# nemo110110/modify-sift-gpu

Hardware: AMD Instinct MI355X
Metric: SIFT images/sec at 1080p (features/sec alongside), 1/2/4/8 MI355X (higher is better)
Workload: dtype f32

## Files before the change

### include/sgpu.h

```cpp
#ifndef SGPU_H
#define SGPU_H
#include <stddef.h>
#include <stdint.h>

#ifdef __cplusplus
extern "C" {
#endif

#define SGPU_OK 0
#define SGPU_EINVAL (-1)
#define SGPU_ENODEV (-2)
#define SGPU_ENOMEM (-3)
#define SGPU_ERANGE (-4)

typedef struct sgpu_options {
    float filter_width_factor;
    float descriptor_window_factor;
    float orientation_window_factor;
    float orientation_gaussian_factor;
    float dog_threshold;
    float edge_threshold;
    int subpixel;
    int max_orientation;
    int fixed_orientation;
// ... 146 lines not shown
#define SGPU_DEBUG_GAUSS_BLOCK 32
#define SGPU_DEBUG_BAND_SHIFT 20
#define SGPU_DEBUG_KEYED_MATCH 64
#define SGPU_DEBUG_FULL_COLUMNS 128
#define SGPU_DEBUG_DESC_DUAL 256
#define SGPU_DEBUG_ORIENT_WAVE 512
#define SGPU_DEBUG_GAUSS_TILE_ALWAYS 1024
#define SGPU_DEBUG_MATCH_REGSTAGE 2048
#define SGPU_DEBUG_PYR_SERIAL 4096
#define SGPU_DEBUG_GAUSS_LONG_BANDS 8192
#define SGPU_DEBUG_DUO_ALWAYS 16384
#define SGPU_DEBUG_DUO_OFF 32768
#define SGPU_DEBUG_GAUSS_TILE_OFF 65536
#define SGPU_DEBUG_DESC_WIDE_OFF 131072
#define SGPU_DEBUG_DESC_WIDE_ALWAYS 262144
#define SGPU_DEBUG_EXTREMA_TILE_OFF 524288

int sgpu_debug_set_flags(sgpu_ctx* ctx, int flags);
#define SGPU_FEATURES_QUEUE 0
#define SGPU_FEATURES_STATIC_ORIENTATION 1
#define SGPU_FEATURES_STATIC_DESCRIPTOR 2
#define SGPU_FEATURES_STATIC 3
int sgpu_debug_set_feature_queue(sgpu_ctx* ctx, int mode);
#define SGPU_TRIO_OFF 0
#define SGPU_TRIO_ON 1
#define SGPU_TRIO_ALWAYS 2
#define SGPU_PAIRS_FRONT 0
#define SGPU_PAIRS_END 1
int sgpu_debug_set_schedule(sgpu_ctx* ctx, int trio, int pairs);
#define SGPU_DUO_STRIPS_RULE 0
#define SGPU_DUO_STRIPS_WAVE 1
#define SGPU_DUO_STRIPS_COOP 2
int sgpu_debug_set_duo_strips(sgpu_ctx* ctx, int mode);
int sgpu_debug_set_match_prune(sgpu_ctx* ctx, int on);
int sgpu_debug_match_plan_stats(const sgpu_ctx* ctx, long long out[4]);
#define SGPU_PLAN_ENTRY_INTS 7
#define SGPU_PLAN_LEVEL 0
#define SGPU_PLAN_TILE 1
#define SGPU_PLAN_TWO 2
#define SGPU_PLAN_TILE_TWO 3
#define SGPU_PLAN_TILE_DUO 4
#define SGPU_PLAN_TILE_DUO_ONE 5
#define SGPU_PLAN_DUO 6
#define SGPU_PLAN_TRIO 7
#define SGPU_PLAN_KINDS 8
int sgpu_debug_pyramid_plan(const sgpu_ctx* ctx, int* out, int cap);
int sgpu_debug_geometry(const sgpu_ctx* ctx, int* n_octaves, int* dims , int max);
int sgpu_debug_gaussian(sgpu_ctx* ctx, int image, int octave, int level, float* out);
int sgpu_debug_candidates(sgpu_ctx* ctx, int* ints, float* floats, int cap, int* n);

#ifdef __cplusplus
}
#endif
#endif
```

### modify-sift-gpu_amd/csrc/sgpu_capi.cpp

```cpp
#include <dlfcn.h>
#include <hip/hip_runtime.h>
#include <rccl/rccl.h>

#include <algorithm>
#include <cmath>
#include <cstdio>
#include <cstdlib>
#include <atomic>
#include <cstring>
#include <string>
#include <vector>

#include "../../include/sgpu.h"
#include "sift_kernels.h"
#include "sift_geom.h"
#include "sift_match_plan.h"
#include "sift_params.h"
#include "sift_pyramid_plan.h"

namespace {

#ifndef SGK_WIDE_DESC_MAX
#define SGK_WIDE_DESC_MAX 8192
#endif
// ... 63 lines not shown
            if (e) (void)hipEventDestroy(e);
        if (stream) (void)hipStreamDestroy(stream);
        if (stream_lo) (void)hipStreamDestroy(stream_lo);
        if (ev_ds) (void)hipEventDestroy(ev_ds);
        if (ev_oct) (void)hipEventDestroy(ev_oct);
        ev_ds = ev_oct = nullptr;
        if (stream_oct) (void)hipStreamDestroy(stream_oct);
        stream = stream_lo = stream_oct = nullptr;
    }
};

constexpr int kMaxParts = 4;
#ifndef SGPU_WAVE_ORIENT_MAX
#define SGPU_WAVE_ORIENT_MAX 16384
#endif
constexpr size_t kWaveOrientationMax = SGPU_WAVE_ORIENT_MAX;

}

struct sgpu_ctx {
    int device = 0;
    hipStream_t stream = nullptr;
    sgpu_options opt{};
    sgp::Schedule sched{};
    sgp::InputPlan plan{};
    int debug_flags = 0;
    bool multi_stream = false;
    bool duo_on = false;
    bool duo_wide = false;
    bool duo_u8 = false;
    int trio_mode = SGPU_TRIO_OFF;
    int duo_plan = SGK_DUO_PLAN;
    int duo_strips = SGPU_DUO_STRIPS_RULE;
    size_t wide_desc_max = SGK_WIDE_DESC_MAX;
    size_t wave_orient_max = kWaveOrientationMax;
    bool unit_input = true;
    bool tile_duo = false;
    int tile_mb = SGK_TILE_MB;
    int env_flags = 0;
    sgk::FeatureQueue fq{};
    bool queue_ori = true, queue_desc = true;
    struct HostOut {
        float* keys = nullptr;
        float* desc = nullptr;
        int cap = 0;
        bool armed = false, active = false, done = false;
    } host_out;
    bool stage_timing = true;
    bool streaming = false;
    std::string err;
    int batch = 0, w = 0, h = 0, nparts = 0;
    std::vector<sgp::Octave> oct;
    size_t staged_bytes = 0;
    std::vector<int64_t> img_off;
    Part part[kMaxParts];
    DevBuf input, all_keys, all_desc, gray, pre;
    DevBuf input2;
    DevBuf duo_trash;
    hipStream_t h2d = nullptr, d2h = nullptr;
    hipEvent_t up_ev[2] = {}, down_ev[2] = {};
    bool gathered = false;
    hipEvent_t ev[T_N + 1] = {};
    float timing[T_N] = {};
    DevBuf m_d1, m_d2, m_s1, m_s2, m_part, m_terms, m_match, m_dist, m_mask, m_loc, m_colpart, m_cols;
    DevBuf m_prune, m_s1c;
    bool match_prune = true;
// ... 169 lines not shown
    if (!pt.ev_ds) {
        for (hipEvent_t& e : pt.ev)
            if (hipEventCreate(&e) != hipSuccess) return SGPU_ENODEV;
        if (hipEventCreateWithFlags(&pt.ev_ds, hipEventDisableTiming) != hipSuccess ||
            hipEventCreateWithFlags(&pt.ev_oct, hipEventDisableTiming) != hipSuccess)
            return SGPU_ENODEV;
    }
    return SGPU_OK;
}

int sgpu_ctx_create(int device, const sgpu_options* opt, sgpu_ctx** out) {
    if (!out) return SGPU_EINVAL;
    *out = nullptr;
    int n = 0;
    if (hipGetDeviceCount(&n) != hipSuccess || n <= 0) return SGPU_ENODEV;
    if (device < 0 || device >= n) return SGPU_EINVAL;
    sgpu_ctx* ctx = new sgpu_ctx();
    ctx->device = device;
    if (hipSetDevice(device) != hipSuccess ||
        hipStreamCreateWithFlags(&ctx->stream, hipStreamNonBlocking) != hipSuccess) {
        delete ctx;
        return SGPU_ENODEV;
    }
    for (int i = 0; i <= T_N; i++) (void)hipEventCreate(&ctx->ev[i]);
    {
        Part* p = ctx->part;
        bool ok = part_streams(p[0], PS_MAIN) == SGPU_OK && part_streams(p[0], PS_OCT) == SGPU_OK &&
                  hipStreamCreateWithFlags(&ctx->h2d, hipStreamNonBlocking) == hipSuccess &&
                  hipStreamCreateWithFlags(&ctx->d2h, hipStreamNonBlocking) == hipSuccess &&
                  part_streams(p[0], PS_LO) == SGPU_OK && part_streams(p[1], PS_OCT) == SGPU_OK &&
                  part_streams(p[2], PS_MAIN) == SGPU_OK && part_streams(p[2], PS_LO) == SGPU_OK &&
                  part_streams(p[1], PS_MAIN) == SGPU_OK && part_streams(p[1], PS_LO) == SGPU_OK;
        ok = ok && sgk::feature_queue_grids(&ctx->fq) == hipSuccess;
        for (int i = 0; ok && i < 2; i++)
            ok = hipEventCreateWithFlags(&ctx->up_ev[i], hipEventDisableTiming) == hipSuccess &&
                 hipEventCreateWithFlags(&ctx->down_ev[i], hipEventDisableTiming) == hipSuccess;
        if (!ok) {
            sgpu_ctx_destroy(ctx);
            return SGPU_ENODEV;
        }
    }
    if (const char* ev = getenv("SGPU_EXACT_DESCRIPTOR"))
        if (ev[0] == '1') ctx->debug_flags |= SGPU_DEBUG_EXACT_DESCRIPTOR;
    if (const char* ev = getenv("SGPU_GAUSS")) {
        if (!strcmp(ev, "block")) ctx->debug_flags |= SGPU_DEBUG_GAUSS_BLOCK;
    }
    if (const char* ev = getenv("SGPU_DUO")) {
        if (!strcmp(ev, "off")) ctx->debug_flags |= SGPU_DEBUG_DUO_OFF;
        if (!strcmp(ev, "always")) ctx->debug_flags |= SGPU_DEBUG_DUO_ALWAYS;
        if (!strcmp(ev, "on")) ctx->duo_on = true;
    }
    if (const char* ev = getenv("SGPU_DUO_WIDE")) {
        if (ev[0] == '1') ctx->duo_wide = true;
    }
    if (const char* ev = getenv("SGPU_DUO_U8")) {
        if (ev[0] == '1') ctx->duo_u8 = true;
    }
    if (const char* ev = getenv("SGPU_DUO_PLAN")) {
        if (!strcmp(ev, "end")) ctx->duo_plan = SGPU_PAIRS_END;
        if (!strcmp(ev, "front")) ctx->duo_plan = SGPU_PAIRS_FRONT;
    }
    if (const char* ev = getenv("SGPU_TRIO")) {
        if (!strcmp(ev, "off")) ctx->trio_mode = SGPU_TRIO_OFF;
        if (!strcmp(ev, "always")) ctx->trio_mode = SGPU_TRIO_ALWAYS;
        if (!strcmp(ev, "on")) ctx->trio_mode = SGPU_TRIO_ON;
    }
    if (const char* ev = getenv("SGPU_GAUSS_BANDS"))
        if (!strcmp(ev, "long")) ctx->debug_flags |= SGPU_DEBUG_GAUSS_LONG_BANDS;
    if (const char* ev = getenv("SGPU_PYR")) {
        if (!strcmp(ev, "serial")) ctx->debug_flags |= SGPU_DEBUG_PYR_SERIAL;
    }
    if (const char* ev = getenv("SGPU_STREAMS")) ctx->multi_stream = !strcmp(ev, "multi");
    if (const char* ev = getenv("SGPU_MATCH"))
        if (!strcmp(ev, "reg")) ctx->debug_flags |= SGPU_DEBUG_MATCH_REGSTAGE;
    if (const char* ev = getenv("SGPU_DESC")) {
        if (!strcmp(ev, "dual")) ctx->debug_flags |= SGPU_DEBUG_DESC_DUAL;
        if (!strcmp(ev, "narrow")) ctx->debug_flags |= SGPU_DEBUG_DESC_WIDE_OFF;
        if (!strcmp(ev, "wide")) ctx->debug_flags |= SGPU_DEBUG_DESC_WIDE_ALWAYS;
    }
    if (const char* ev = getenv("SGPU_GAUSS_TILE")) {
        if (!strcmp(ev, "off")) ctx->debug_flags |= SGPU_DEBUG_GAUSS_TILE_OFF;
        if (!strcmp(ev, "always")) ctx->debug_flags |= SGPU_DEBUG_GAUSS_TILE_ALWAYS;
    }
    if (const char* ev = getenv("SGPU_WIDE_DESC_MAX"))
        if (atoll(ev) >= 0) ctx->wide_desc_max = (size_t)atoll(ev);
    if (const char* ev = getenv("SGPU_WAVE_ORIENT_MAX"))
        if (atoll(ev) >= 0) ctx->wave_orient_max = (size_t)atoll(ev);
    if (const char* ev = getenv("SGPU_EXTREMA")) {
        if (!strcmp(ev, "wave")) ctx->debug_flags |= SGPU_DEBUG_EXTREMA_TILE_OFF;
// ... 278 lines not shown
    auto rec = [&](int i, hipStream_t s_) -> hipError_t {
        return pt.events ? hipEventRecord(pt.ev[i], s_) : hipSuccess;
    };
    HIPCHK(ctx, rec(0, st));
    const size_t img_elems = (size_t)stride * h;
    const uint8_t* src8 = is_f32 ? nullptr : (const uint8_t*)src_in + (size_t)pt.img0 * img_elems;
    const float* srcf = is_f32 ? (const float*)src_in + (size_t)pt.img0 * img_elems : nullptr;

    float* pyr = pt.pyr.as<float>();
    const int rc_ops = build_level_ops(ctx, pt, src8, srcf, stride, st);
    if (rc_ops != SGPU_OK) return rc_ops;
    const sgpyr::Rules R = pyramid_rules(ctx, pt);
    sgpyr::plan_pyramid(pt.levels.data(), (int)pt.levels.size(), R, OpSupport{pt.ops.data()}, pt.plan);
    const int rc_trash = pt.plan.trash ? ensure_gauss_trash(ctx) : SGPU_OK;
    if (rc_trash != SGPU_OK) return rc_trash;
    const bool side = pt.plan.side;
    float* const trash = ctx->duo_trash.as<float>();
    pt.gauss_launches = 0;
    for (const sgpyr::Launch& l : pt.plan.launches) {
        const hipStream_t s_ = l.side ? pt.stream_oct : st;
        const sgk::LevelOp& a = pt.ops[l.op[0]];
        const sgk::LevelOp& b = pt.ops[std::max(l.op[1], 0)];
        const sgk::LevelOp& c = pt.ops[std::max(l.op[2], 0)];
        int nl = 1;
        if (l.wait_ds) HIPCHK(ctx, hipStreamWaitEvent(s_, pt.ev_ds, 0));
        switch (l.kind) {
            case sgpyr::kLevel: HIPCHK(ctx, sgk::launch_gauss_op(a, s_, R.wave_rows, R.long_bands)); break;
            case sgpyr::kTile: HIPCHK(ctx, sgk::launch_gauss_tile(a, s_)); break;
            case sgpyr::kTwo: HIPCHK(ctx, sgk::launch_gauss_two(a, b, s_, R.wave_rows, R.long_bands, &nl)); break;
            case sgpyr::kTileTwo: HIPCHK(ctx, sgk::launch_gauss_tile_two(a, b, s_, &nl)); break;
            case sgpyr::kTileDuo: HIPCHK(ctx, sgk::launch_gauss_tile_duo(a, b, s_)); break;
            case sgpyr::kTileDuoOne: HIPCHK(ctx, sgk::launch_gauss_tile_duo_one(a, b, c, s_, &nl)); break;
            case sgpyr::kDuo:
                HIPCHK(ctx, sgk::launch_gauss_duo(a, b, s_, R.wave_rows, trash, ctx->duo_strips));
                break;
            case sgpyr::kTrio: HIPCHK(ctx, sgk::launch_gauss_trio(a, b, c, s_, R.wave_rows, trash)); break;
            default: return ctx->fail(SGPU_EINVAL, "unknown pyramid launch kind");
        }
        pt.gauss_launches += nl;
        if (l.rec_ds) HIPCHK(ctx, hipEventRecord(pt.ev_ds, st));
    }
    if (side) {
        HIPCHK(ctx, hipEventRecord(pt.ev_oct, pt.stream_oct));
        HIPCHK(ctx, hipStreamWaitEvent(st, pt.ev_oct, 0));
    }
    HIPCHK(ctx, rec(1, st));

    if (!pt.one_stream)
        HIPCHK(ctx, sgk::launch_zero(pt.row_count.as<uint32_t>(), (size_t)pt.total_rows,
                                     pt.mask.as<uint32_t>(), (size_t)moff, nullptr, 0, st));
    const bool ext_tiles = !(ctx->debug_flags & SGPU_DEBUG_EXTREMA_TILE_OFF) &&
                           ((ctx->debug_flags & SGPU_DEBUG_GAUSS_TILE_ALWAYS) ||
                            4ll * fp.oct[0].wa * fp.oct[0].h * n <= ((long long)ctx->tile_mb << 20));
    HIPCHK(ctx, sgk::launch_extrema(pyr, pt.mask.as<uint32_t>(), pt.row_count.as<uint32_t>(),
                                    fp, st, ext_tiles));
    if (O.feature_count_threshold > 0)
        HIPCHK(ctx, sgk::launch_limit_rows(pt.row_count.as<uint32_t>(), fp,
                                           O.feature_count_threshold, O.truncate_method, st));
    HIPCHK(ctx, rec(7, st));
    HIPCHK(ctx, sgk::launch_scan(pt.row_count.as<uint32_t>(), pt.row_base.as<uint32_t>(),
                                 pt.total_rows, pt.scan_tmp.as<uint32_t>(), st));
    HIPCHK(ctx, rec(2, st));

    if (!pt.one_stream) {
        st = pt.stream_lo;
        HIPCHK(ctx, hipStreamWaitEvent(st, pt.ev[2], 0));
    }
// ... 1493 lines not shown
    out[0] = (long long)plan.items.size();
    out[1] = (long long)plan.sides.size();
    out[2] = tiles;
    out[3] = chunks;
    return SGPU_OK;
}

static_assert(SGPU_PLAN_KINDS == sgpyr::kKinds && SGPU_PLAN_TRIO == sgpyr::kTrio &&
              SGPU_PLAN_TILE_DUO_ONE == sgpyr::kTileDuoOne, "sgpu.h and sift_pyramid_plan.h agree");
int sgpu_debug_pyramid_plan(const sgpu_ctx* ctx, int* out, int cap) {
    if (!ctx || ctx->batch <= 0 || cap < 0 || (cap > 0 && !out)) return SGPU_EINVAL;
    const Part& pt = ctx->part[0];
    const int n = (int)pt.plan.launches.size();
    for (int e = 0; e < n && (e + 1) * SGPU_PLAN_ENTRY_INTS <= cap; e++) {
        const sgpyr::Launch& l = pt.plan.launches[e];
        int* p = out + e * SGPU_PLAN_ENTRY_INTS;
        p[0] = l.kind;
        for (int j = 0; j < 3; j++) {
            p[1 + 2 * j] = l.op[j] < 0 ? -1 : pt.levels[l.op[j]].o;
            p[2 + 2 * j] = l.op[j] < 0 ? -1 : pt.levels[l.op[j]].k;
        }
    }
    return n;
}

static_assert(SGPU_DUO_STRIPS_RULE == sgk::kDuoStripsRule && SGPU_DUO_STRIPS_WAVE == sgk::kDuoStripsWave &&
              SGPU_DUO_STRIPS_COOP == sgk::kDuoStripsCoop, "sgpu.h and sift_kernels.h agree");
int sgpu_debug_set_duo_strips(sgpu_ctx* ctx, int mode) {
    if (!ctx || mode < SGPU_DUO_STRIPS_RULE || mode > SGPU_DUO_STRIPS_COOP) return SGPU_EINVAL;
    ctx->duo_strips = mode;
    return SGPU_OK;
}

int sgpu_debug_set_feature_queue(sgpu_ctx* ctx, int mode) {
    if (!ctx || mode < SGPU_FEATURES_QUEUE || mode > SGPU_FEATURES_STATIC) return SGPU_EINVAL;
    ctx->queue_ori = !(mode & SGPU_FEATURES_STATIC_ORIENTATION);
    ctx->queue_desc = !(mode & SGPU_FEATURES_STATIC_DESCRIPTOR);
    return SGPU_OK;
}

int sgpu_debug_set_schedule(sgpu_ctx* ctx, int trio, int pairs) {
    if (!ctx || trio < SGPU_TRIO_OFF || trio > SGPU_TRIO_ALWAYS || pairs < SGPU_PAIRS_FRONT ||
        pairs > SGPU_PAIRS_END)
        return SGPU_EINVAL;
    ctx->trio_mode = trio;
    ctx->duo_plan = pairs;
    return SGPU_OK;
}

int sgpu_debug_geometry(const sgpu_ctx* ctx, int* n_octaves, int* dims, int max) {
    if (!ctx || !n_octaves) return SGPU_EINVAL;
    *n_octaves = (int)ctx->oct.size();
    for (int o = 0; o < (int)ctx->oct.size() && o < max; o++) {
        dims[3 * o] = ctx->oct[o].w;
        dims[3 * o + 1] = ctx->oct[o].h;
        dims[3 * o + 2] = ctx->oct[o].wa;
    }
    return SGPU_OK;
}

int sgpu_debug_gaussian(sgpu_ctx* ctx, int image, int octave, int level, float* out) {
    if (!ctx || image < 0 || image >= ctx->batch || octave < 0 ||
        octave >= (int)ctx->oct.size() || level < 0 || level >= ctx->sched.level_num)
        return SGPU_EINVAL;
    HIPCHK(ctx, hipSetDevice(ctx->device));
    const Part& pt = ctx->part[ctx->part_of(image)];
// ... 63 lines not shown
```

### modify-sift-gpu_amd/csrc/sift_gauss_duo.hip

```cpp
#include <cstdint>
#include <cstdlib>
#include <cstring>
#include <utility>

#include "sift_gauss_coop_plan.h"
#include "sift_gauss_ring.h"
#include "sift_kernels.h"
#include "sift_pyramid_plan.h"

#pragma clang diagnostic ignored "-Winline-asm"

namespace sgk {
namespace {

using namespace gring;

#ifndef SGK_DUO_INTERLEAVE
#define SGK_DUO_INTERLEAVE 1
#endif
constexpr bool kDuoInterleave = SGK_DUO_INTERLEAVE != 0;
#ifndef SGK_DUO_EXP
#define SGK_DUO_EXP 0
#endif
#ifndef SGK_DUO_X4
#define SGK_DUO_X4 1
#endif
constexpr int kDuoWaves = 4;
constexpr int kMidSlot = 256;
static_assert(kDuoWaves == coop::kWaves && 2 * coop::kWaveCols == kMidSlot, "cooperative geometry");

__device__ __forceinline__ void coop_barrier() {
    asm volatile("" ::: "memory");
    wait_lgkm0();
    __builtin_amdgcn_s_barrier();
    asm volatile("" ::: "memory");
}

// ... 490 lines not shown
        return e ? atoi(e) : SGK_DUO_NIN;
    }();
    return v == 5 ? 5 : v == 4 ? 4 : 7;
}
static int duo_bands_env() {
    static const int v = [] {
        const char* e = getenv("SGPU_DUO_BANDS");
        return e ? atoi(e) : 0;
    }();
    return v;
}
#ifndef SGK_DUO_WAVES
#define SGK_DUO_WAVES 4096
#endif
static long long duo_waves_target() {
    static const long long v = [] {
        const char* e = getenv("SGPU_DUO_WAVES");
        return e && atoll(e) > 0 ? atoll(e) : (long long)SGK_DUO_WAVES;
    }();
    return v;
}

template <int FWA, int FWB>
constexpr bool kDuoCoopCompiled = !(FWA == 17 && FWB == 21);
#ifndef SGK_DUO_COOP_RULE
#define SGK_DUO_COOP_RULE 1
#endif
#ifndef SGK_DUO_COOP_MAXW
#define SGK_DUO_COOP_MAXW 1920
#endif
template <int FWA, int FWB>
constexpr bool kDuoCoopRule = SGK_DUO_COOP_RULE != 0 && SGK_DUO_EXP == 0 && kDuoCoopCompiled<FWA, FWB>;

template <int FWA, int FWB, bool U8, int DS, bool COOP>
hipError_t duo_launch_form(const LevelOp& a, const LevelOp& b, hipStream_t stream, int rows_hint,
                           float* trash) {
    using G = DuoGeom<FWA, FWB>;
    DuoJob J{};
    J.src = a.src;
    J.src8 = a.src_u8;
    J.zero = a.zero;
    J.src_stride = a.src_stride;
    J.src_img = a.src_img_stride;
    J.dst1 = a.dst;
    J.dst2 = b.dst;
    J.dst_img = a.dst_img_stride;
    J.W = a.w;
    J.H = a.h;
    J.ta = a.taps;
    J.tb = b.taps;
    const LevelOp& dl = DS == 2 ? b : a;
    J.ds = dl.ds_dst;
    J.dsw = dl.ds_w;
    J.dsh = dl.ds_h;
    J.ds_img = dl.ds_img_stride;
    J.strips = COOP ? coop::strips(a.w, FWB) : (a.w + G::SW - 1) / G::SW;
    const long long per_band = (long long)J.strips * a.batch * (COOP ? kDuoWaves : 1);
    int nsy = 1;
    const long long want = duo_waves_target();
    if (rows_hint > 0) {
        nsy = (a.h + rows_hint - 1) / rows_hint;
    } else if (duo_bands_env() > 0) {
        nsy = std::min(duo_bands_env(), std::max(1, a.h / 64));
    } else if (per_band < want) {
        nsy = (int)std::min<long long>((want + per_band - 1) / per_band, std::max(1, a.h / 64));
    }
    int rows = (a.h + nsy - 1) / nsy;
    rows = (rows + 7) / 8 * 8;
    J.nsy = (a.h + rows - 1) / rows;
    J.rows_per_band = rows;
    J.total_waves = (int)(per_band * J.nsy);
    J.trash = trash;
    const unsigned nb = (unsigned)((J.total_waves + kDuoWaves - 1) / kDuoWaves);
    if constexpr (U8)
        hipLaunchKernelGGL((k_gauss_duo<FWA, FWB, 2, true, DS, COOP>), dim3(nb), dim3(64 * kDuoWaves), 0, stream, J);
    else if constexpr (COOP)
        hipLaunchKernelGGL((k_gauss_duo<FWA, FWB, 7, false, DS, true>), dim3(nb), dim3(64 * kDuoWaves), 0, stream, J);
    else if (duo_nin() == 5)
        hipLaunchKernelGGL((k_gauss_duo<FWA, FWB, 5, false, DS, false>), dim3(nb), dim3(64 * kDuoWaves), 0, stream, J);
    else if (duo_nin() == 4)
        hipLaunchKernelGGL((k_gauss_duo<FWA, FWB, 4, false, DS, false>), dim3(nb), dim3(64 * kDuoWaves), 0, stream, J);
    else
        hipLaunchKernelGGL((k_gauss_duo<FWA, FWB, 7, false, DS, false>), dim3(nb), dim3(64 * kDuoWaves), 0, stream, J);
    return hipGetLastError();
}

template <int FWA, int FWB, bool U8, int DS>
hipError_t duo_launch(const LevelOp& a, const LevelOp& b, hipStream_t stream, int rows_hint,
                      float* trash, int strips) {
    if constexpr (kDuoCoopCompiled<FWA, FWB>) {
        const bool rule = kDuoCoopRule<FWA, FWB> && a.w <= SGK_DUO_COOP_MAXW &&
                          coop::fewer_lane_columns(a.w, FWB);
        if (strips == kDuoStripsCoop || (strips == kDuoStripsRule && rule))
            return duo_launch_form<FWA, FWB, U8, DS, true>(a, b, stream, rows_hint, trash);
    }
    return duo_launch_form<FWA, FWB, U8, DS, false>(a, b, stream, rows_hint, trash);
}

}

bool gauss_duo_supported(const LevelOp& a, const LevelOp& b) {
    const bool u8 = a.src_u8 != nullptr;
    const bool ds = a.ds_dst != nullptr, dsb = b.ds_dst != nullptr;
    const bool widths = sgpyr::duo_widths(a.fw, b.fw, u8, ds, dsb);
    const bool dsb_ok = dsb && widths && (b.w % 2) == 0 && b.ds_w * 2 == b.w &&
                        (b.ds_h == (b.h + 1) / 2 || b.ds_h == b.h / 2) &&
                        b.ds_img_stride >= (long long)b.ds_w * b.ds_h;
    const bool dsa_ok = (a.w % 2) == 0 && a.ds_w * 2 == a.w && a.ds_h == (a.h + 1) / 2 &&
                        a.ds_img_stride >= (long long)a.ds_w * a.ds_h;
    const bool pair = widths && (!dsb || dsb_ok) && (u8 || dsb || !ds || dsa_ok);
    const bool src_ok = u8 ? (!a.src && (a.src_stride % 4) == 0 && (a.src_img_stride % 4) == 0 &&
                              ((uintptr_t)a.src_u8 % 4) == 0)
                           : (a.src && a.src_stride >= a.w);
    const bool b_zeroes = (b.zero.n[0] | b.zero.n[1] | b.zero.n[2]) != 0;
    const bool a_zeroes = (a.zero.n[0] | a.zero.n[1] | a.zero.n[2]) != 0;
    return pair && src_ok && !b_zeroes && (u8 || !a_zeroes) && (!b.ds_dst || dsb_ok) &&
           b.src == a.dst && !b.src_u8 && a.w == b.w && a.h == b.h && a.batch == b.batch &&
           a.w >= 8 && a.h >= 8 && (a.w % 4) == 0 && b.src_stride == a.w &&
           a.dst_img_stride == b.dst_img_stride && b.src_img_stride == a.dst_img_stride &&
           a.dst_img_stride >= (long long)a.w * a.h;
}

hipError_t launch_gauss_duo(const LevelOp& a, const LevelOp& b, hipStream_t stream, int rows_hint,
                            float* trash, int strips) {
    if (!trash || !gauss_duo_supported(a, b)) return hipErrorInvalidValue;
    if (a.src_u8) return duo_launch<13, 11, true, 0>(a, b, stream, rows_hint, trash, strips);
    if (a.ds_dst) return duo_launch<17, 21, false, 1>(a, b, stream, rows_hint, trash, strips);
    if (b.ds_dst) return duo_launch<13, 17, false, 2>(a, b, stream, rows_hint, trash, strips);
#define SGK_DUO(A, B) \
    if (a.fw == A && b.fw == B) return duo_launch<A, B, false, 0>(a, b, stream, rows_hint, trash, strips);
    SGK_DUO(11, 13) SGK_DUO(21, 25)
#undef SGK_DUO
    return hipErrorInvalidValue;
}

}
```

### modify-sift-gpu_amd/csrc/sift_kernels.h

```cpp
#pragma once
#include <hip/hip_runtime.h>
#include <stdint.h>

namespace sgk {

constexpr int kMaxLevels = 16;
constexpr int kMaxOctaves = 16;

struct Taps { float k[33]; };

struct OctaveDesc {
    int w, h, wa;
    int nwords;
    long long gauss_off;
    long long level_stride;
    long long mask_off;
    long long mask_level_stride;
};

struct FeatureParams {
    int batch, n_octaves, d;
    int rows_per_image;
    int row_off[kMaxOctaves];
    float level_sigma[kMaxLevels];
// ... 12 lines not shown
    uint32_t* p[3] = {nullptr, nullptr, nullptr};
    size_t n[3] = {0, 0, 0};
};

hipError_t launch_gauss(const float* src, const uint8_t* src_u8, int src_stride,
                        long long src_img_stride, float* dst, long long dst_img_stride,
                        int w, int h, int fw, const Taps& taps, int batch,
                        float* ds_dst, int ds_w, int ds_h, long long ds_img_stride,
                        hipStream_t stream, int wave_rows = -1, bool long_bands = false,
                        const ZeroJob& zero = ZeroJob{});

struct LevelOp {
    const float* src;
    const uint8_t* src_u8;
    int src_stride;
    long long src_img_stride;
    float* dst;
    long long dst_img_stride;
    int w, h, fw;
    Taps taps;
    int batch;
    float* ds_dst;
    int ds_w, ds_h;
    long long ds_img_stride;
    ZeroJob zero;
};
hipError_t launch_gauss_op(const LevelOp& op, hipStream_t stream, int wave_rows,
                           bool long_bands = false);
hipError_t launch_gauss_two(const LevelOp& a, const LevelOp& b, hipStream_t stream, int wave_rows,
                            bool long_bands = false, int* launches = nullptr);

constexpr size_t kGaussDuoTrashBytes = 1024 * 3072;
constexpr int kDuoStripsRule = 0, kDuoStripsWave = 1, kDuoStripsCoop = 2;
bool gauss_duo_supported(const LevelOp& a, const LevelOp& b);
hipError_t launch_gauss_duo(const LevelOp& a, const LevelOp& b, hipStream_t stream, int rows_hint,
                            float* trash, int strips = kDuoStripsRule);

constexpr size_t kGaussTrioTrashBytes = 1024 * 4096;
bool gauss_trio_supported(const LevelOp& a, const LevelOp& b, const LevelOp& c);
hipError_t launch_gauss_trio(const LevelOp& a, const LevelOp& b, const LevelOp& c,
                             hipStream_t stream, int rows_hint, float* trash);

bool gauss_tile_supported(const LevelOp& op);
hipError_t launch_gauss_tile(const LevelOp& op, hipStream_t stream);
hipError_t launch_gauss_tile_two(const LevelOp& a, const LevelOp& b, hipStream_t stream,
                                 int* launches = nullptr);
bool gauss_tile_duo_supported(const LevelOp& a, const LevelOp& b);
hipError_t launch_gauss_tile_duo(const LevelOp& a, const LevelOp& b, hipStream_t stream);
hipError_t launch_gauss_tile_duo_one(const LevelOp& a, const LevelOp& b, const LevelOp& c,
                                     hipStream_t stream, int* launches = nullptr);

hipError_t launch_first_octave_input(const float* src, const uint8_t* src_u8, int stride,
                                     long long src_img_stride, int tw, int h, int fo, float* dst,
                                     int dw, int dh, long long dst_img_stride, int batch,
                                     hipStream_t stream);

hipError_t launch_color_to_gray(const uint8_t* src, int n, int w, int h, int stride,
                                int channels, bool bgr, float* dst, hipStream_t stream);

hipError_t launch_extrema(const float* pyr, uint32_t* mask, uint32_t* row_count,
                          const FeatureParams& fp, hipStream_t stream, bool tiles = false);

size_t scan_tmp_words(size_t n);
hipError_t launch_zero(uint32_t* a, size_t na, uint32_t* b, size_t nb, uint32_t* c, size_t nc,
                       hipStream_t stream);
hipError_t launch_scan(const uint32_t* in, uint32_t* out, size_t n, uint32_t* tmp,
                       hipStream_t stream);

constexpr int kQueueCounters = 8;
// ... 154 lines not shown
```

### modify-sift-gpu_amd/python/sgpu.py

```python
from __future__ import annotations

import contextlib
import ctypes
import os
import subprocess

import numpy as np

from sgpu_types import SgpuOptions, default_options

PKG = os.path.dirname(os.path.dirname(os.path.abspath(__file__)))
LIB_PATH = os.environ.get("SGPU_LIB_PATH") or os.path.join(PKG, "lib", "libsiftgpu.so")

SGPU_OK, SGPU_EINVAL, SGPU_ENODEV, SGPU_ENOMEM, SGPU_ERANGE = 0, -1, -2, -3, -4
SGPU_INPUT_HOST, SGPU_INPUT_DEVICE, SGPU_INPUT_STAGED = 0, 1, 2

C_API = [
    "sgpu_default_options", "sgpu_parse_args", "sgpu_ctx_create", "sgpu_ctx_destroy",
    "sgpu_ctx_set_options", "sgpu_last_error", "sgpu_device_count", "sgpu_extract",
    "sgpu_extract_f32", "sgpu_stage_input", "sgpu_feature_count", "sgpu_feature_total", "sgpu_copy_features",
    "sgpu_device_features", "sgpu_match", "sgpu_quantize_descriptors", "sgpu_last_timing",
    "sgpu_debug_geometry", "sgpu_debug_gaussian", "sgpu_debug_candidates",
    "sgpu_debug_set_flags", "sgpu_comm_unique_id", "sgpu_comm_init", "sgpu_comm_allgather_i32",
    "sgpu_comm_allreduce_f64", "sgpu_extract_keypoints", "sgpu_match_guided", "sgpu_extract_color",
    "sgpu_match_shard_begin", "sgpu_match_shard_end", "sgpu_match_sharded",
    "sgpu_extract_stream", "sgpu_host_alloc", "sgpu_host_free", "sgpu_reserve",
    "sgpu_debug_alloc_count", "sgpu_last_pyramid_launches", "sgpu_set_stage_timing",
    "sgpu_set_host_output", "sgpu_debug_set_schedule", "sgpu_debug_set_match_prune",
    "sgpu_quantize_descriptors_gpu", "sgpu_feature_descriptors_u8", "sgpu_copy_features_u8",
    "sgpu_match_batch", "sgpu_match_images", "sgpu_debug_match_plan_stats",
    "sgpu_debug_set_duo_strips", "sgpu_debug_pyramid_plan", "sgpu_debug_set_feature_queue",
    "sgpu_match_batch_guided", "sgpu_match_images_guided",
    "sgpu_estimate_batch", "sgpu_estimate_images",
]

PLAN_KINDS = ("level", "tile", "two", "tile_two", "tile_duo", "tile_duo_one", "duo", "trio")

_LIB = None


def build():
    subprocess.check_call(["make", "-C", PKG, "-j8"])


def lib():
    global _LIB
    if _LIB is None:
        if not os.path.exists(LIB_PATH):
            raise RuntimeError(f"{LIB_PATH} missing: build it with `make -C {PKG}`")
        L = ctypes.CDLL(LIB_PATH)
        P, c = ctypes.POINTER, ctypes
        vp = c.c_void_p
        L.sgpu_default_options.argtypes = [P(SgpuOptions)]
        L.sgpu_parse_args.argtypes = [P(SgpuOptions), c.c_int, P(c.c_char_p), P(c.c_int)]
        L.sgpu_ctx_create.argtypes = [c.c_int, P(SgpuOptions), P(vp)]
        L.sgpu_ctx_destroy.argtypes = [vp]
        L.sgpu_ctx_set_options.argtypes = [vp, P(SgpuOptions)]
        L.sgpu_last_error.argtypes = [vp]
        L.sgpu_last_error.restype = c.c_char_p
        L.sgpu_extract.argtypes = [vp, vp, c.c_int, c.c_int, c.c_int, c.c_int, c.c_int]
        L.sgpu_stage_input.argtypes = [vp, vp, c.c_int, c.c_int, c.c_int, c.c_int]
        L.sgpu_reserve.argtypes = [vp, c.c_int, c.c_int, c.c_int, c.c_int]
        L.sgpu_debug_alloc_count.argtypes = []
        L.sgpu_debug_alloc_count.restype = c.c_longlong
        L.sgpu_last_pyramid_launches.argtypes = [vp, P(c.c_int)]
        L.sgpu_set_stage_timing.argtypes = [vp, c.c_int]
        L.sgpu_set_host_output.argtypes = [vp, vp, vp, c.c_int]
        L.sgpu_extract_f32.argtypes = [vp, vp, c.c_int, c.c_int, c.c_int, c.c_int, c.c_int]
        L.sgpu_feature_count.argtypes = [vp, c.c_int]
        L.sgpu_feature_total.argtypes = [vp]
        L.sgpu_feature_total.restype = c.c_int64
        L.sgpu_copy_features.argtypes = [vp, c.c_int, vp, vp]
        L.sgpu_device_features.argtypes = [vp, P(vp), P(vp), P(vp)]
        L.sgpu_match.argtypes = [vp, vp, c.c_int, vp, c.c_int, c.c_float, c.c_float, c.c_int,
                                 c.c_int, vp, c.c_int]
        L.sgpu_match_guided.argtypes = [vp, vp, c.c_int, vp, c.c_int, vp, vp, vp, vp, c.c_float,
                                        c.c_float, c.c_float, c.c_float, c.c_int, c.c_int, vp,
                                        c.c_int]
        L.sgpu_extract_color.argtypes = [vp, vp, c.c_int, c.c_int, c.c_int, c.c_int, c.c_int, c.c_int]
        L.sgpu_quantize_descriptors.argtypes = [vp, c.c_size_t, vp]
        L.sgpu_last_timing.argtypes = [vp, vp, c.c_int]
        L.sgpu_debug_set_flags.argtypes = [vp, c.c_int]
        L.sgpu_debug_set_schedule.argtypes = [vp, c.c_int, c.c_int]
        L.sgpu_debug_set_match_prune.argtypes = [vp, c.c_int]
        L.sgpu_debug_set_duo_strips.argtypes = [vp, c.c_int]
        L.sgpu_debug_set_feature_queue.argtypes = [vp, c.c_int]
        L.sgpu_debug_geometry.argtypes = [vp, P(c.c_int), vp, c.c_int]
        L.sgpu_debug_gaussian.argtypes = [vp, c.c_int, c.c_int, c.c_int, vp]
        L.sgpu_debug_candidates.argtypes = [vp, vp, vp, c.c_int, P(c.c_int)]
        L.sgpu_extract_keypoints.argtypes = [vp, c.c_int, vp, c.c_int, c.c_int]
        L.sgpu_comm_unique_id.argtypes = [vp, c.c_int]
        L.sgpu_comm_init.argtypes = [vp, c.c_int, c.c_int, vp, c.c_int]
        L.sgpu_comm_allgather_i32.argtypes = [vp, vp, c.c_int, vp]
        L.sgpu_comm_allreduce_f64.argtypes = [vp, vp, c.c_int, c.c_int]
        L.sgpu_match_shard_begin.argtypes = [vp, vp, c.c_int, c.c_int, vp, c.c_int, c.c_float,
                                             c.c_float, c.c_int, vp, vp, c.c_int]
        L.sgpu_match_shard_end.argtypes = [vp, c.c_int, c.c_int, vp, c.c_int, c.c_int, c.c_float,
                                           c.c_float, c.c_int, c.c_int, vp]
        L.sgpu_match_sharded.argtypes = [vp, vp, c.c_int, c.c_int, vp, c.c_int, c.c_float,
                                         c.c_float, c.c_int, c.c_int, vp, c.c_int]
        L.sgpu_extract_stream.argtypes = [vp, P(vp), c.c_int, c.c_int, c.c_int, c.c_int, c.c_int,
                                          vp, vp, c.c_int64, vp]
        L.sgpu_host_alloc.argtypes = [c.c_size_t]
        L.sgpu_host_alloc.restype = vp
        L.sgpu_host_free.argtypes = [vp]
        L.sgpu_quantize_descriptors_gpu.argtypes = [vp, vp, c.c_size_t, vp, c.c_int]
        L.sgpu_feature_descriptors_u8.argtypes = [vp, P(vp)]
        L.sgpu_copy_features_u8.argtypes = [vp, c.c_int, vp]
        L.sgpu_match_batch.argtypes = [vp, vp, vp, c.c_int, vp, c.c_int, c.c_float, c.c_float,
                                       c.c_int, c.c_int, vp, c.c_int64, vp, c.c_int]
        L.sgpu_match_images.argtypes = [vp, vp, c.c_int, c.c_float, c.c_float, c.c_int, c.c_int,
                                        vp, c.c_int64, vp]
        L.sgpu_match_batch_guided.argtypes = [vp, vp, vp, vp, c.c_int, vp, c.c_int, vp, vp,
                                              c.c_float, c.c_float, c.c_float, c.c_float,
                                              c.c_int, c.c_int, vp, c.c_int64, vp, c.c_int]
        L.sgpu_match_images_guided.argtypes = [vp, vp, c.c_int, vp, vp, c.c_float, c.c_float,
                                               c.c_float, c.c_float, c.c_int, c.c_int, vp,
                                               c.c_int64, vp]
# ... 556 lines not shown
    DEBUG_PARTS2, DEBUG_PARTS4, DEBUG_TINY_CAP, DEBUG_FUSED_MATCH = 1, 2, 4, 8
    DEBUG_EXACT_DESCRIPTOR = 16
    DEBUG_GAUSS_BLOCK = 32
    DEBUG_BAND_SHIFT = 20
    DEBUG_KEYED_MATCH = 64
    DEBUG_FULL_COLUMNS = 128
    DEBUG_DESC_DUAL = 256
    DEBUG_ORIENT_WAVE = 512
    DEBUG_GAUSS_TILE_ALWAYS = 1024
    DEBUG_MATCH_REGSTAGE = 2048
    DEBUG_PYR_SERIAL = 4096
    DEBUG_GAUSS_LONG_BANDS = 8192
    DEBUG_DUO_ALWAYS = 16384
    DEBUG_DUO_OFF = 32768
    DEBUG_GAUSS_TILE_OFF = 65536
    DEBUG_DESC_WIDE_OFF = 131072
    DEBUG_DESC_WIDE_ALWAYS = 262144
    DEBUG_EXTREMA_TILE_OFF = 524288

    def set_debug_flags(self, flags: int):
        self._check(lib().sgpu_debug_set_flags(self._ctx, flags), "sgpu_debug_set_flags")

    TRIO_OFF, TRIO_ON, TRIO_ALWAYS = 0, 1, 2
    PAIRS_FRONT, PAIRS_END = 0, 1

    def set_schedule(self, trio: int = 0, pairs: int = 1):
        self._check(lib().sgpu_debug_set_schedule(self._ctx, trio, pairs), "sgpu_debug_set_schedule")

    STRIPS_RULE, STRIPS_WAVE, STRIPS_COOP = 0, 1, 2

    def set_duo_strips(self, mode: int = 0):
        self._check(lib().sgpu_debug_set_duo_strips(self._ctx, mode), "sgpu_debug_set_duo_strips")

    FEATURES_QUEUE, FEATURES_STATIC_ORIENTATION, FEATURES_STATIC_DESCRIPTOR, FEATURES_STATIC = 0, 1, 2, 3

    def set_feature_queue(self, mode: int = 0):
        self._check(lib().sgpu_debug_set_feature_queue(self._ctx, mode), "sgpu_debug_set_feature_queue")

    def set_match_prune(self, on: bool = True):
        self._check(lib().sgpu_debug_set_match_prune(self._ctx, int(bool(on))),
                    "sgpu_debug_set_match_prune")

    def match_plan_stats(self):
        out = np.zeros(4, np.int64)
        self._check(lib().sgpu_debug_match_plan_stats(self._ctx, out.ctypes.data),
                    "sgpu_debug_match_plan_stats")
        return dict(zip(["items", "sides", "max_tiles", "max_chunks"], out.tolist()))

    @contextlib.contextmanager
    def exact_descriptors(self):
        self.set_debug_flags(self.DEBUG_EXACT_DESCRIPTOR)
        try:
            yield self
        finally:
            self.set_debug_flags(0)

    def geometry(self):
        n = ctypes.c_int(0)
        dims = np.zeros(48, np.int32)
        lib().sgpu_debug_geometry(self._ctx, ctypes.byref(n), dims.ctypes.data, 16)
        return [tuple(dims[3 * i:3 * i + 3]) for i in range(n.value)]

    def gaussian(self, image, octave, level):
        w, h, wa = self.geometry()[octave]
        out = np.zeros(wa * h, np.float32)
        self._check(lib().sgpu_debug_gaussian(self._ctx, image, octave, level, out.ctypes.data),
# ... 12 lines not shown
```

Baseline: 19080.

## Choose duo Gaussian band count by occupancy-aware round cost model

Adds a band-planning model that queries per-kernel occupancy and CU count at context creation, then picks the number of row bands for cooperative duo Gaussian launches by minimising a cost over full and partial rounds, including halo warm-up rows. This replaces the simple wave-target heuristic for the default coop path and aims to reduce tail underutilisation against the redundant halo work of extra bands. It also adds an optional 4-input ring variant for two filter pairs and debug/env controls. The fixed cost constants tuned for partial rounds may not fit every shape.

```diff
diff --git a/include/sgpu.h b/include/sgpu.h
--- a/include/sgpu.h
+++ b/include/sgpu.h
@@ -202,6 +202,11 @@
 #define SGPU_DUO_STRIPS_WAVE 1
 #define SGPU_DUO_STRIPS_COOP 2
 int sgpu_debug_set_duo_strips(sgpu_ctx* ctx, int mode);
+#define SGPU_DUO_BANDS_RULE 0
+#define SGPU_DUO_BANDS_WAVES 1
+#define SGPU_DUO_BANDS_ROUNDS 2
+int sgpu_debug_set_duo_bands(sgpu_ctx* ctx, int mode, int capacity);
+int sgpu_debug_duo_occupancy(sgpu_ctx* ctx, int* out, int cap);
 int sgpu_debug_set_match_prune(sgpu_ctx* ctx, int on);
 int sgpu_debug_match_plan_stats(const sgpu_ctx* ctx, long long out[4]);
 #define SGPU_PLAN_ENTRY_INTS 7
diff --git a/modify-sift-gpu_amd/csrc/sgpu_capi.cpp b/modify-sift-gpu_amd/csrc/sgpu_capi.cpp
--- a/modify-sift-gpu_amd/csrc/sgpu_capi.cpp
+++ b/modify-sift-gpu_amd/csrc/sgpu_capi.cpp
@@ -119,6 +119,7 @@
     int trio_mode = SGPU_TRIO_OFF;
     int duo_plan = SGK_DUO_PLAN;
     int duo_strips = SGPU_DUO_STRIPS_RULE;
+    sgk::DuoBands duo_bands;
     size_t wide_desc_max = SGK_WIDE_DESC_MAX;
     size_t wave_orient_max = kWaveOrientationMax;
     bool unit_input = true;
@@ -354,6 +355,7 @@
                   part_streams(p[2], PS_MAIN) == SGPU_OK && part_streams(p[2], PS_LO) == SGPU_OK &&
                   part_streams(p[1], PS_MAIN) == SGPU_OK && part_streams(p[1], PS_LO) == SGPU_OK;
         ok = ok && sgk::feature_queue_grids(&ctx->fq) == hipSuccess;
+        ok = ok && sgk::gauss_duo_occupancy(&ctx->duo_bands) == hipSuccess;
         for (int i = 0; ok && i < 2; i++)
             ok = hipEventCreateWithFlags(&ctx->up_ev[i], hipEventDisableTiming) == hipSuccess &&
                  hipEventCreateWithFlags(&ctx->down_ev[i], hipEventDisableTiming) == hipSuccess;
@@ -377,6 +379,13 @@
     }
     if (const char* ev = getenv("SGPU_DUO_U8")) {
         if (ev[0] == '1') ctx->duo_u8 = true;
+    }
+    if (const char* ev = getenv("SGPU_DUO_BAND_RULE")) {
+        if (!strcmp(ev, "waves")) ctx->duo_bands.mode = sgk::kDuoBandsWaves;
+        if (!strcmp(ev, "rounds")) ctx->duo_bands.mode = sgk::kDuoBandsRounds;
+    }
+    if (const char* ev = getenv("SGPU_DUO_NIN")) {
+        if (atoi(ev) == 4 || atoi(ev) == 7) ctx->duo_bands.coop_ring = atoi(ev);
     }
     if (const char* ev = getenv("SGPU_DUO_PLAN")) {
         if (!strcmp(ev, "end")) ctx->duo_plan = SGPU_PAIRS_END;
@@ -721,7 +730,8 @@
             case sgpyr::kTileDuo: HIPCHK(ctx, sgk::launch_gauss_tile_duo(a, b, s_)); break;
             case sgpyr::kTileDuoOne: HIPCHK(ctx, sgk::launch_gauss_tile_duo_one(a, b, c, s_, &nl)); break;
             case sgpyr::kDuo:
-                HIPCHK(ctx, sgk::launch_gauss_duo(a, b, s_, R.wave_rows, trash, ctx->duo_strips));
+                HIPCHK(ctx, sgk::launch_gauss_duo(a, b, s_, R.wave_rows, trash, ctx->duo_strips,
+                                                  &ctx->duo_bands));
                 break;
             case sgpyr::kTrio: HIPCHK(ctx, sgk::launch_gauss_trio(a, b, c, s_, R.wave_rows, trash)); break;
             default: return ctx->fail(SGPU_EINVAL, "unknown pyramid launch kind");
@@ -2281,6 +2291,22 @@
     return SGPU_OK;
 }
 
+static_assert(SGPU_DUO_BANDS_RULE == sgk::kDuoBandsRule && SGPU_DUO_BANDS_WAVES == sgk::kDuoBandsWaves &&
+              SGPU_DUO_BANDS_ROUNDS == sgk::kDuoBandsRounds, "sgpu.h and sift_kernels.h agree");
+int sgpu_debug_set_duo_bands(sgpu_ctx* ctx, int mode, int capacity) {
+    if (!ctx || mode < SGPU_DUO_BANDS_RULE || mode > SGPU_DUO_BANDS_ROUNDS || capacity < 0) return SGPU_EINVAL;
+    ctx->duo_bands.mode = mode;
+    ctx->duo_bands.capacity = mode == SGPU_DUO_BANDS_ROUNDS ? capacity : 0;
+    return SGPU_OK;
+}
+
+int sgpu_debug_duo_occupancy(sgpu_ctx* ctx, int* out, int cap) {
+    if (!ctx || !out || cap < 1 + sgk::kDuoKernels) return SGPU_EINVAL;
+    out[0] = ctx->duo_bands.cus;
+    for (int i = 0; i < sgk::kDuoKernels; i++) out[1 + i] = ctx->duo_bands.per_cu[i];
+    return 1 + sgk::kDuoKernels;
+}
+
 int sgpu_debug_set_feature_queue(sgpu_ctx* ctx, int mode) {
     if (!ctx || mode < SGPU_FEATURES_QUEUE || mode > SGPU_FEATURES_STATIC) return SGPU_EINVAL;
     ctx->queue_ori = !(mode & SGPU_FEATURES_STATIC_ORIENTATION);
diff --git a/modify-sift-gpu_amd/csrc/sift_gauss_band_plan.h b/modify-sift-gpu_amd/csrc/sift_gauss_band_plan.h
--- /dev/null
+++ b/modify-sift-gpu_amd/csrc/sift_gauss_band_plan.h
@@ -0,0 +1,59 @@
+#pragma once
+
+namespace sgk {
+namespace band {
+
+constexpr int kMinRows = 64;
+constexpr int kRowAlign = 8;
+
+constexpr int kG0Three = 220;
+constexpr int kG0Four = 50;
+
+struct Plan {
+    int nsy;
+    int rows;
+};
+
+constexpr int max_bands(int h) { return h / kMinRows > 1 ? h / kMinRows : 1; }
+constexpr int warm_rows(int fwa, int fwb) { return 2 * (fwa / 2) + 2 * (fwb / 2) + 2; }
+
+constexpr Plan split(int h, int n) {
+    int rows = (h + n - 1) / n;
+    rows = (rows + kRowAlign - 1) / kRowAlign * kRowAlign;
+    return Plan{(h + rows - 1) / rows, rows};
+}
+
+constexpr Plan by_waves(int h, long long per_band, long long want) {
+    int n = 1;
+    if (per_band > 0 && per_band < want) {
+        const long long need = (want + per_band - 1) / per_band;
+        n = need < max_bands(h) ? (int)need : max_bands(h);
+    }
+    return split(h, n);
+}
+
+constexpr long long cost(const Plan& p, long long units, int warm, long long C, int g0) {
+    const long long U = units * p.nsy;
+    const long long full = U / C, part = U % C;
+    const long long rounds = 1000 * C * full + (part ? g0 * C + (1000 - g0) * part : 0);
+    return (long long)(p.rows + warm) * rounds;
+}
+
+constexpr Plan by_rounds(int h, long long units, int warm, long long C, int g0) {
+    if (units < 1) units = 1;
+    if (C < 1) C = 1;
+    Plan best = split(h, 1);
+    long long cbest = cost(best, units, warm, C, g0);
+    for (int n = 2; n <= max_bands(h); n++) {
+        const Plan p = split(h, n);
+        const long long c = cost(p, units, warm, C, g0);
+        if (c < cbest || (c == cbest && p.nsy < best.nsy)) {
+            best = p;
+            cbest = c;
+        }
+    }
+    return best;
+}
+
+}
+}
diff --git a/modify-sift-gpu_amd/csrc/sift_gauss_duo.hip b/modify-sift-gpu_amd/csrc/sift_gauss_duo.hip
--- a/modify-sift-gpu_amd/csrc/sift_gauss_duo.hip
+++ b/modify-sift-gpu_amd/csrc/sift_gauss_duo.hip
@@ -3,6 +3,7 @@
 #include <cstring>
 #include <utility>
 
+#include "sift_gauss_band_plan.h"
 #include "sift_gauss_coop_plan.h"
 #include "sift_gauss_ring.h"
 #include "sift_kernels.h"
@@ -559,9 +560,47 @@
 template <int FWA, int FWB>
 constexpr bool kDuoCoopRule = SGK_DUO_COOP_RULE != 0 && SGK_DUO_EXP == 0 && kDuoCoopCompiled<FWA, FWB>;
 
+template <int FWA, int FWB, bool U8>
+constexpr bool kDuoCoopRing4 = !U8 && ((FWA == 13 && FWB == 17) || (FWA == 11 && FWB == 13));
+constexpr int kDuoCoopRing = 7;
+
+template <int FWA, int FWB>
+constexpr int kDuoPairSlot = 5 * (FWA == 13 && FWB == 11 ? 0 : FWA == 17 && FWB == 21 ? 1
+                                  : FWA == 13 && FWB == 17 ? 2 : FWA == 11 && FWB == 13 ? 3 : 4);
+constexpr int duo_form_slot(bool coop, int nin) {
+    return coop ? (nin == 4 ? 4 : 3) : (nin == 5 ? 1 : nin == 4 ? 2 : 0);
+}
+
+template <int FWA, int FWB, bool U8, bool COOP>
+constexpr bool kDuoRoundsRule = COOP && !U8 && SGK_DUO_EXP == 0;
+
+template <int FWA, int FWB, int NIN, bool U8, int DS, bool COOP>
+hipError_t duo_occupancy_of(int* per_cu) {
+    return hipOccupancyMaxActiveBlocksPerMultiprocessor(per_cu, k_gauss_duo<FWA, FWB, NIN, U8, DS, COOP>,
+                                                        64 * kDuoWaves, 0);
+}
+template <int FWA, int FWB, bool U8, int DS>
+hipError_t duo_pair_occupancy(DuoBands* b) {
+    int* t = b->per_cu + kDuoPairSlot<FWA, FWB>;
+    hipError_t e = hipSuccess;
+    if constexpr (U8) {
+        e = duo_occupancy_of<FWA, FWB, 2, true, DS, false>(&t[duo_form_slot(false, 7)]);
+        if (e == hipSuccess) e = duo_occupancy_of<FWA, FWB, 2, true, DS, true>(&t[duo_form_slot(true, 7)]);
+    } else {
+        if (duo_nin() == 5) e = duo_occupancy_of<FWA, FWB, 5, false, DS, false>(&t[duo_form_slot(false, 5)]);
+        else if (duo_nin() == 4) e = duo_occupancy_of<FWA, FWB, 4, false, DS, false>(&t[duo_form_slot(false, 4)]);
+        else e = duo_occupancy_of<FWA, FWB, 7, false, DS, false>(&t[duo_form_slot(false, 7)]);
+        if constexpr (kDuoCoopCompiled<FWA, FWB>)
+            if (e == hipSuccess) e = duo_occupancy_of<FWA, FWB, 7, false, DS, true>(&t[duo_form_slot(true, 7)]);
+        if constexpr (kDuoCoopRing4<FWA, FWB, U8>)
+            if (e == hipSuccess) e = duo_occupancy_of<FWA, FWB, 4, false, DS, true>(&t[duo_form_slot(true, 4)]);
+    }
+    return e;
+}
+
 template <int FWA, int FWB, bool U8, int DS, bool COOP>
 hipError_t duo_launch_form(const LevelOp& a, const LevelOp& b, hipStream_t stream, int rows_hint,
-                           float* trash) {
+                           float* trash, const DuoBands* bands) {
     using G = DuoGeom<FWA, FWB>;
     DuoJob J{};
     J.src = a.src;
@@ -583,29 +622,43 @@
     J.ds_img = dl.ds_img_stride;
     J.strips = COOP ? coop::strips(a.w, FWB) : (a.w + G::SW - 1) / G::SW;
     const long long per_band = (long long)J.strips * a.batch * (COOP ? kDuoWaves : 1);
-    int nsy = 1;
-    const long long want = duo_waves_target();
+    const int ring = bands && bands->coop_ring ? bands->coop_ring : kDuoCoopRing;
+    const int nin = U8 ? 2 : !COOP ? duo_nin() : (kDuoCoopRing4<FWA, FWB, U8> && ring == 4 ? 4 : 7);
+    const int mode = bands ? bands->mode : kDuoBandsWaves;
+    band::Plan P;
     if (rows_hint > 0) {
-        nsy = (a.h + rows_hint - 1) / rows_hint;
+        P = band::split(a.h, (a.h + rows_hint - 1) / rows_hint);
     } else if (duo_bands_env() > 0) {
-        nsy = std::min(duo_bands_env(), std::max(1, a.h / 64));
-    } else if (per_band < want) {
-        nsy = (int)std::min<long long>((want + per_band - 1) / per_band, std::max(1, a.h / 64));
+        P = band::split(a.h, std::min(duo_bands_env(), band::max_bands(a.h)));
+    } else if (mode == kDuoBandsRounds || (mode == kDuoBandsRule && kDuoRoundsRule<FWA, FWB, U8, COOP>)) {
+        const int per_cu = bands->per_cu[kDuoPairSlot<FWA, FWB> + duo_form_slot(COOP, U8 ? 7 : nin)];
+        const long long cap = mode == kDuoBandsRounds && bands->capacity > 0
+                                  ? bands->capacity : (long long)per_cu * bands->cus;
+        if (per_cu <= 0 || cap <= 0) return hipErrorInvalidValue;
+        const long long units = COOP ? per_band / kDuoWaves : (per_band + kDuoWaves - 1) / kDuoWaves;
+        P = band::by_rounds(a.h, units, band::warm_rows(FWA, FWB), cap,
+                            per_cu >= 4 ? band::kG0Four : band::kG0Three);
+    } else {
+        P = band::by_waves(a.h, per_band, duo_waves_target());
     }
-    int rows = (a.h + nsy - 1) / nsy;
-    rows = (rows + 7) / 8 * 8;
-    J.nsy = (a.h + rows - 1) / rows;
-    J.rows_per_band = rows;
+    J.nsy = P.nsy;
+    J.rows_per_band = P.rows;
     J.total_waves = (int)(per_band * J.nsy);
     J.trash = trash;
     const unsigned nb = (unsigned)((J.total_waves + kDuoWaves - 1) / kDuoWaves);
-    if constexpr (U8)
+    if constexpr (U8) {
         hipLaunchKernelGGL((k_gauss_duo<FWA, FWB, 2, true, DS, COOP>), dim3(nb), dim3(64 * kDuoWaves), 0, stream, J);
-    else if constexpr (COOP)
+    } else if constexpr (COOP) {
+        if constexpr (kDuoCoopRing4<FWA, FWB, U8>) {
+            if (nin == 4) {
+                hipLaunchKernelGGL((k_gauss_duo<FWA, FWB, 4, false, DS, true>), dim3(nb), dim3(64 * kDuoWaves), 0, stream, J);
+                return hipGetLastError();
+            }
+        }
         hipLaunchKernelGGL((k_gauss_duo<FWA, FWB, 7, false, DS, true>), dim3(nb), dim3(64 * kDuoWaves), 0, stream, J);
-    else if (duo_nin() == 5)
+    } else if (nin == 5)
         hipLaunchKernelGGL((k_gauss_duo<FWA, FWB, 5, false, DS, false>), dim3(nb), dim3(64 * kDuoWaves), 0, stream, J);
-    else if (duo_nin() == 4)
+    else if (nin == 4)
         hipLaunchKernelGGL((k_gauss_duo<FWA, FWB, 4, false, DS, false>), dim3(nb), dim3(64 * kDuoWaves), 0, stream, J);
     else
         hipLaunchKernelGGL((k_gauss_duo<FWA, FWB, 7, false, DS, false>), dim3(nb), dim3(64 * kDuoWaves), 0, stream, J);
@@ -614,14 +667,14 @@
 
 template <int FWA, int FWB, bool U8, int DS>
 hipError_t duo_launch(const LevelOp& a, const LevelOp& b, hipStream_t stream, int rows_hint,
-                      float* trash, int strips) {
+                      float* trash, int strips, const DuoBands* bands) {
     if constexpr (kDuoCoopCompiled<FWA, FWB>) {
         const bool rule = kDuoCoopRule<FWA, FWB> && a.w <= SGK_DUO_COOP_MAXW &&
                           coop::fewer_lane_columns(a.w, FWB);
         if (strips == kDuoStripsCoop || (strips == kDuoStripsRule && rule))
-            return duo_launch_form<FWA, FWB, U8, DS, true>(a, b, stream, rows_hint, trash);
+            return duo_launch_form<FWA, FWB, U8, DS, true>(a, b, stream, rows_hint, trash, bands);
     }
-    return duo_launch_form<FWA, FWB, U8, DS, false>(a, b, stream, rows_hint, trash);
+    return duo_launch_form<FWA, FWB, U8, DS, false>(a, b, stream, rows_hint, trash, bands);
 }
 
 }
@@ -648,14 +701,27 @@
            a.dst_img_stride >= (long long)a.w * a.h;
 }
 
+hipError_t gauss_duo_occupancy(DuoBands* bands) {
+    int dev = 0;
+    hipError_t e = hipGetDevice(&dev);
+    if (e == hipSuccess) e = hipDeviceGetAttribute(&bands->cus, hipDeviceAttributeMultiprocessorCount, dev);
+    if (e == hipSuccess) e = duo_pair_occupancy<13, 11, true, 0>(bands);
+    if (e == hipSuccess) e = duo_pair_occupancy<17, 21, false, 1>(bands);
+    if (e == hipSuccess) e = duo_pair_occupancy<13, 17, false, 2>(bands);
+    if (e == hipSuccess) e = duo_pair_occupancy<11, 13, false, 0>(bands);
+    if (e == hipSuccess) e = duo_pair_occupancy<21, 25, false, 0>(bands);
+    if (e == hipSuccess && bands->cus <= 0) e = hipErrorInvalidValue;
+    return e;
+}
+
 hipError_t launch_gauss_duo(const LevelOp& a, const LevelOp& b, hipStream_t stream, int rows_hint,
-                            float* trash, int strips) {
+                            float* trash, int strips, const DuoBands* bands) {
     if (!trash || !gauss_duo_supported(a, b)) return hipErrorInvalidValue;
-    if (a.src_u8) return duo_launch<13, 11, true, 0>(a, b, stream, rows_hint, trash, strips);
-    if (a.ds_dst) return duo_launch<17, 21, false, 1>(a, b, stream, rows_hint, trash, strips);
-    if (b.ds_dst) return duo_launch<13, 17, false, 2>(a, b, stream, rows_hint, trash, strips);
+    if (a.src_u8) return duo_launch<13, 11, true, 0>(a, b, stream, rows_hint, trash, strips, bands);
+    if (a.ds_dst) return duo_launch<17, 21, false, 1>(a, b, stream, rows_hint, trash, strips, bands);
+    if (b.ds_dst) return duo_launch<13, 17, false, 2>(a, b, stream, rows_hint, trash, strips, bands);
 #define SGK_DUO(A, B) \
-    if (a.fw == A && b.fw == B) return duo_launch<A, B, false, 0>(a, b, stream, rows_hint, trash, strips);
+    if (a.fw == A && b.fw == B) return duo_launch<A, B, false, 0>(a, b, stream, rows_hint, trash, strips, bands);
     SGK_DUO(11, 13) SGK_DUO(21, 25)
 #undef SGK_DUO
     return hipErrorInvalidValue;
diff --git a/modify-sift-gpu_amd/csrc/sift_kernels.h b/modify-sift-gpu_amd/csrc/sift_kernels.h
--- a/modify-sift-gpu_amd/csrc/sift_kernels.h
+++ b/modify-sift-gpu_amd/csrc/sift_kernels.h
@@ -68,9 +68,20 @@
 
 constexpr size_t kGaussDuoTrashBytes = 1024 * 3072;
 constexpr int kDuoStripsRule = 0, kDuoStripsWave = 1, kDuoStripsCoop = 2;
+constexpr int kDuoBandsRule = 0, kDuoBandsWaves = 1, kDuoBandsRounds = 2;
+constexpr int kDuoKernels = 25;
+struct DuoBands {
+    int mode = kDuoBandsRule;
+    int capacity = 0;
+    int coop_ring = 0;
+    int cus = 0;
+    int per_cu[kDuoKernels] = {};
+};
+hipError_t gauss_duo_occupancy(DuoBands* bands);
 bool gauss_duo_supported(const LevelOp& a, const LevelOp& b);
 hipError_t launch_gauss_duo(const LevelOp& a, const LevelOp& b, hipStream_t stream, int rows_hint,
-                            float* trash, int strips = kDuoStripsRule);
+                            float* trash, int strips = kDuoStripsRule,
+                            const DuoBands* bands = nullptr);
 
 constexpr size_t kGaussTrioTrashBytes = 1024 * 4096;
 bool gauss_trio_supported(const LevelOp& a, const LevelOp& b, const LevelOp& c);
diff --git a/modify-sift-gpu_amd/python/sgpu.py b/modify-sift-gpu_amd/python/sgpu.py
--- a/modify-sift-gpu_amd/python/sgpu.py
+++ b/modify-sift-gpu_amd/python/sgpu.py
@@ -32,6 +32,7 @@
     "sgpu_debug_set_duo_strips", "sgpu_debug_pyramid_plan", "sgpu_debug_set_feature_queue",
     "sgpu_match_batch_guided", "sgpu_match_images_guided",
     "sgpu_estimate_batch", "sgpu_estimate_images",
+    "sgpu_debug_set_duo_bands", "sgpu_debug_duo_occupancy",
 ]
 
 PLAN_KINDS = ("level", "tile", "two", "tile_two", "tile_duo", "tile_duo_one", "duo", "trio")
@@ -84,6 +85,8 @@
         L.sgpu_debug_set_schedule.argtypes = [vp, c.c_int, c.c_int]
         L.sgpu_debug_set_match_prune.argtypes = [vp, c.c_int]
         L.sgpu_debug_set_duo_strips.argtypes = [vp, c.c_int]
+        L.sgpu_debug_set_duo_bands.argtypes = [vp, c.c_int, c.c_int]
+        L.sgpu_debug_duo_occupancy.argtypes = [vp, P(c.c_int), c.c_int]
         L.sgpu_debug_set_feature_queue.argtypes = [vp, c.c_int]
         L.sgpu_debug_geometry.argtypes = [vp, P(c.c_int), vp, c.c_int]
         L.sgpu_debug_gaussian.argtypes = [vp, c.c_int, c.c_int, c.c_int, vp]
@@ -706,6 +709,18 @@
     def set_duo_strips(self, mode: int = 0):
         self._check(lib().sgpu_debug_set_duo_strips(self._ctx, mode), "sgpu_debug_set_duo_strips")
 
+    BANDS_RULE, BANDS_WAVES, BANDS_ROUNDS = 0, 1, 2
+
+    def set_duo_bands(self, mode: int = 0, capacity: int = 0):
+        self._check(lib().sgpu_debug_set_duo_bands(self._ctx, mode, capacity), "sgpu_debug_set_duo_bands")
+
+    def duo_occupancy(self):
+        buf = (ctypes.c_int * 64)()
+        n = lib().sgpu_debug_duo_occupancy(self._ctx, buf, 64)
+        if n < 1:
+            raise RuntimeError("sgpu_debug_duo_occupancy failed")
+        return buf[0], list(buf[1:n])
+
     FEATURES_QUEUE, FEATURES_STATIC_ORIENTATION, FEATURES_STATIC_DESCRIPTOR, FEATURES_STATIC = 0, 1, 2, 3
 
     def set_feature_queue(self, mode: int = 0):
```

Result: no change. 19200 (median of 3 runs) (+0.6%).
